# 3decomp/poissbox

Measured on AMD Instinct MI355X. Metric: CG iter/s and DoF-updates/s at 512^3; achieved HBM GB/s vs peak, higher is better.
Workload: dtype f64

## Files before the change

### include/poissbox_gpu.h

```cpp
#ifndef POISSBOX_GPU_H
#define POISSBOX_GPU_H

#include <stdint.h>

#ifdef __cplusplus
extern "C" {
#endif

#define PB_VERSION_MAJOR 0
#define PB_VERSION_MINOR 2

enum pb_error {
  PB_OK = 0,
  PB_ERR_ARG = 1,
  PB_ERR_HIP = 2,
  PB_ERR_COMM = 3,
  PB_ERR_ALLOC = 4,
  PB_ERR_UNSUPPORTED = 5,
  PB_ERR_STATE = 6
};

typedef struct pb_ctx pb_ctx;
typedef struct pb_grid pb_grid;
typedef struct pb_vec pb_vec;
// ... 181 lines not shown
int pb_solve_fgmres(pb_op* A, pb_op* P, const pb_ksp_opts* opts, const pb_ksp_fgmres_opts* fg,
                    const pb_vec* b, pb_vec* x, pb_ksp_result* res, double* history,
                    int64_t history_cap);
int pb_pc_mg_opts_default(pb_pc_mg_opts* opts);
int pb_pc_mg_opts_parse(pb_pc_mg_opts* opts, int argc, const char* const* argv);
int pb_ksp_pc_mg_set_opts(pb_ksp* ksp, const pb_pc_mg_opts* opts);
int pb_ksp_pc_mg_get_opts(const pb_ksp* ksp, pb_pc_mg_opts* opts);
int pb_solve_mg(pb_op* A, pb_op* P, const pb_ksp_opts* opts, const pb_pc_mg_opts* mg,
                const pb_vec* b, pb_vec* x, pb_ksp_result* res, double* history,
                int64_t history_cap);
int pb_ksp_chebyshev_get_eigenvalues(pb_ksp* ksp, double* emin, double* emax, int* estimated);
int pb_tridiag_extreme_eigenvalues(int n, const double* diag, const double* off, double* lo,
                                   double* hi);
int pb_ksp_pc_apply(pb_ksp* ksp, const pb_vec* r, pb_vec* z);
int pb_ksp_pc_levels(const pb_ksp* ksp, int* levels);
int pb_ksp_pc_set_coefficient_from(pb_ksp* ksp, const pb_op* C);
int pb_ksp_pc_get_coefficient_from(const pb_ksp* ksp, const pb_op** C);
int pb_ksp_guess_form(pb_ksp* ksp, const pb_vec* b, pb_vec* x);
int pb_ksp_guess_update(pb_ksp* ksp, const pb_vec* b, const pb_vec* x);
int pb_ksp_guess_reset(pb_ksp* ksp);
int pb_ksp_guess_size(const pb_ksp* ksp, int* curl, int* maxl);
int pb_solve(pb_op* A, pb_op* P, const pb_ksp_opts* opts, const pb_vec* b, pb_vec* x,
             pb_ksp_result* res, double* history, int64_t history_cap);

int pb_tdma_batched(pb_ctx* ctx, int64_t n, int64_t nbatch, int64_t line_stride,
                    int64_t elem_stride, const double* a, double* b, const double* c, double* d,
                    int periodic);
int pb_tdma_sweeps_batched(pb_ctx* ctx, int64_t n, int64_t nbatch, int64_t line_stride,
                           int64_t elem_stride, const double* a, double* b, const double* c,
                           double* d, int which);
// ... 38 lines not shown
```

### poissbox_amd/_lib.py

```python
import ctypes as C
import os
import subprocess

_HERE = os.path.dirname(os.path.abspath(__file__))
LIB_PATH = os.environ.get("PB_LIB") or os.path.join(_HERE, "libpoissbox_gpu.so")

c_i64 = C.c_int64
c_d = C.c_double
c_p = C.c_void_p
P_d = C.POINTER(C.c_double)
P_i64 = C.POINTER(C.c_int64)


class PbError(RuntimeError):
    def __init__(self, code, msg, where):
        super().__init__(f"{where} failed (code {code}): {msg}")
        self.code = code


class KspOpts(C.Structure):
    _fields_ = [("rtol", c_d), ("atol", c_d), ("dtol", c_d), ("max_it", c_i64),
                ("ksp_type", C.c_int), ("pc_type", C.c_int), ("nullspace", C.c_int),
                ("monitor", C.c_int), ("converged_reason", C.c_int), ("check_every", C.c_int),
                ("mg_levels", C.c_int), ("mg_coarse_its", C.c_int), ("sor_omega", c_d),
# ... 116 lines not shown
    "pb_ksp_fgmres_opts_default": [C.POINTER(KspFgmresOpts)],
    "pb_ksp_fgmres_opts_parse": [C.POINTER(KspFgmresOpts), C.c_int, C.POINTER(C.c_char_p)],
    "pb_ksp_fgmres_set_opts": [c_p, C.POINTER(KspFgmresOpts)],
    "pb_ksp_fgmres_get_opts": [c_p, C.POINTER(KspFgmresOpts)],
    "pb_solve_fgmres": [c_p, c_p, C.POINTER(KspOpts), C.POINTER(KspFgmresOpts), c_p, c_p,
                        C.POINTER(KspResult), P_d, c_i64],
    "pb_pc_mg_opts_default": [C.POINTER(PcMgOpts)],
    "pb_pc_mg_opts_parse": [C.POINTER(PcMgOpts), C.c_int, C.POINTER(C.c_char_p)],
    "pb_ksp_pc_mg_set_opts": [c_p, C.POINTER(PcMgOpts)],
    "pb_ksp_pc_mg_get_opts": [c_p, C.POINTER(PcMgOpts)],
    "pb_solve_mg": [c_p, c_p, C.POINTER(KspOpts), C.POINTER(PcMgOpts), c_p, c_p,
                    C.POINTER(KspResult), P_d, c_i64],
    "pb_tridiag_extreme_eigenvalues": [C.c_int, P_d, P_d, P_d, P_d],
    "pb_ksp_pc_apply": [c_p, c_p, c_p],
    "pb_ksp_pc_levels": [c_p, C.POINTER(C.c_int)],
    "pb_ksp_pc_set_coefficient_from": [c_p, c_p],
    "pb_ksp_pc_get_coefficient_from": [c_p, C.POINTER(c_p)],
    "pb_solve": [c_p, c_p, C.POINTER(KspOpts), c_p, c_p, C.POINTER(KspResult), P_d, c_i64],
    "pb_tdma_batched": [c_p, c_i64, c_i64, c_i64, c_i64, c_p, c_p, c_p, c_p, C.c_int],
    "pb_pcr_alpha_batched": [c_p, c_i64, c_i64, c_i64, c_i64, c_d, c_p],
    "pb_compact_grad": [c_p, P_d, c_p, C.POINTER(c_p)],
    "pb_compact_div": [c_p, P_d, C.POINTER(c_p), c_p],
    "pb_compact_interp": [c_p, C.c_int, c_p, c_p],
    "pb_compact_lapl": [c_p, P_d, c_p, c_p],
    "pb_compact_lapl_fast": [c_p, P_d, c_p, c_p],
    "pb_compact_grad_fast": [c_p, P_d, c_p, C.POINTER(c_p)],
    "pb_compact_div_fast": [c_p, P_d, C.POINTER(c_p), c_p],
    "pb_compact_interp_fast": [c_p, C.c_int, c_p, c_p],
    "pb_compact_1d_batched": [c_p, C.c_int, C.c_int, c_d, c_i64, c_i64, c_i64, c_i64, c_p, c_p],
    "pb_tdma_sweeps_batched": [c_p, c_i64, c_i64, c_i64, c_i64, c_p, c_p, c_p, c_p, C.c_int],
# ... 44 lines not shown
```

### poissbox_amd/api.py

```python
import ctypes as C

import numpy as np

from . import _lib as L

STAR7, COMPACT, ASSEMBLED27 = 0, 1, 2
VARCOEF = 3
COEF_ARITHMETIC, COEF_HARMONIC = 0, 1
PC_NONE, PC_JACOBI, PC_SOR, PC_MG, PC_FFT = 0, 1, 2, 3, 4
KSP_CG, KSP_PREONLY, KSP_RICHARDSON, KSP_CHEBYSHEV, KSP_FGMRES, KSP_PIPECG = 0, 1, 2, 3, 4, 5
FGMRES_REFINE_NEVER, FGMRES_REFINE_ALWAYS = 0, 2
MG_LEVELS_RICHARDSON, MG_LEVELS_CHEBYSHEV = 0, 1
KSP_NORM_DEFAULT, KSP_NORM_NONE, KSP_NORM_PRECONDITIONED = -1, 0, 1
KSP_NORM_UNPRECONDITIONED, KSP_NORM_NATURAL = 2, 3
MG_LEVELS_SOR, MG_LEVELS_JACOBI = 0, 1

REASONS = {0: "CONVERGED_ITERATING", 2: "CONVERGED_RTOL", 3: "CONVERGED_ATOL",
           4: "CONVERGED_ITS", -3: "DIVERGED_ITS", -4: "DIVERGED_DTOL",
           -8: "DIVERGED_INDEFINITE_PC", -9: "DIVERGED_NANORINF",
           -10: "DIVERGED_INDEFINITE_MAT", -5: "DIVERGED_BREAKDOWN",
           7: "CONVERGED_HAPPY_BREAKDOWN"}


def _i64_3(v):
# ... 562 lines not shown

    def chebyshev_eigenvalues(self):
        lo, hi, est = C.c_double(), C.c_double(), C.c_int()
        L.call("pb_ksp_chebyshev_get_eigenvalues", self.h, C.byref(lo), C.byref(hi), C.byref(est))
        return lo.value, hi.value, bool(est.value)

    def pc_apply(self, r, z):
        L.call("pb_ksp_pc_apply", self.h, r.h, z.h)

    @property
    def pc_levels(self):
        v = C.c_int(0)
        L.call("pb_ksp_pc_levels", self.h, C.byref(v))
        return v.value

    def pc_set_coefficient_from(self, op):
        L.call("pb_ksp_pc_set_coefficient_from", self.h, op.h if op is not None else None)
        self._pc_coef = op

    def pc_coefficient_from(self):
        h = C.c_void_p()
        L.call("pb_ksp_pc_get_coefficient_from", self.h, C.byref(h))
        if not h.value:
            return None
        op = getattr(self, "_pc_coef", None)
        assert op is not None and op.h.value == h.value
        return op

    def destroy(self):
        if self.h:
# ... 101 lines not shown
```

### poissbox_amd/csrc/pb_internal.hpp

```cpp
#pragma once

#include <hip/hip_runtime.h>
#include <rccl/rccl.h>
#include <rocprofiler-sdk-roctx/roctx.h>

#include <cstdint>
#include <cstdio>
#include <deque>
#include <map>
#include <string>
#include <functional>
#include <vector>

#include "poissbox_gpu.h"

namespace pb {

int set_error(int code, const char* fmt, ...);

#define PB_HIP(call)                                                                    \
  do {                                                                                  \
    hipError_t e_ = (call);                                                             \
    if (e_ != hipSuccess)                                                               \
      return ::pb::set_error(PB_ERR_HIP, "%s:%d %s: %s", __FILE__, __LINE__, #call,     \
// ... 248 lines not shown
int launch_mac_grad(pb_grid* g, const MacCoef& c, const double* p, double s, double* const u[3],
                    bool project, const StencilPlanes& gp, int mode);
int launch_mac_div(pb_grid* g, const MacCoef& c, double s, const double* const u[3], double* out,
                   const StencilPlanes& gp, int mode);
int launch_aij_seams(pb_grid* g, const Star& s, const double* x, const double* glo,
                     const double* ghi, double* y);
struct CgState;
int launch_mg_sor(pb_grid* g, const Star& s, double* x, const double* b, const StencilPlanes& gp,
                  double omega, int color, int first, const int* skip,
                  const CgState* sums_st = nullptr, int* nparts = nullptr);
bool sor_sweep2_supported(const pb_grid* g);
int launch_sor_sweep2(pb_grid* g, const Star& s, const double* xin, const double* b, double* xout,
                      double omega, int c1, const int* skip, const CgState* sums_st = nullptr,
                      int* nparts = nullptr);
int launch_presmooth_restrict(pb_grid* g, const Star& s, const pb_grid* cg, const double* b,
                              double* xout, double* bc, double omega, const int* skip);
int launch_post_sweep(pb_grid* g, const Star& s, const pb_grid* cg, const double* xs,
                      const double* xc, const double* b, double* xout, double omega,
                      const int* skip, const CgState* sums_st = nullptr, int* nparts = nullptr,
                      const double* xc_full = nullptr);
int launch_presmooth_residual(pb_grid* g, const Star& s, const double* b, double* x, double* res,
                              double omega, const int* skip);
int launch_mg_residual(pb_grid* g, const Star& s, const double* x, const double* b,
                       const StencilPlanes& gp, double* res, const int* skip);
int launch_mg_poly(pb_grid* g, const Star& s, const double* y, const double* yp, const double* r,
                   const double* b, double scale, double omega, double* y_out, double* r_out,
                   const int* skip);

struct CgState {
  double beta, betaold, dpi, dpiold, alpha, alpha_prev, mu, dp, ttol, rnorm0;
  double pa[3];
  double rtol, atol, dtol, dinv, ntot;
  int64_t it, its, max_it, nhist, pend_iter, pend_count;
  int64_t nlog;
  int reason, done, pc, nullspace, defer_x;
// ... 248 lines not shown
int launch_cheb_update(pb_grid* g, const Star& s, const double* y, const double* ym1,
                       const double* q, const double* b, double* y_out, double* r_out,
                       const StencilPlanes& gp, const CgState* st, double scale, bool sums,
                       int* nparts, int part_off = 0);
int launch_cheb_x(pb_grid* g, const double* y, const double* ym1, const double* q, double* y_out,
                  const CgState* st, double scale);
int launch_pre_scale_sum(pb_grid* g, const double* src, double* dst, double dinv, int* nparts);
int launch_pre_shift(pb_grid* g, double* x, double ntot);

struct Mg;
int mg_create(pb_grid* g, const double deltas[3], int pc_type, int levels_req, int coarse_its,
              double omega, Mg** out);
int mg_apply(Mg* mg, const double* r, double* z, const int* skip = nullptr,
             const CgState* sums_st = nullptr, int* nparts = nullptr);
int mg_levels(const Mg* mg);
struct MgSmoother {
  int ksp = 0, pc = 0, nu = 1;
  double rich_scale = 1.0, emin = 0.0, emax = 0.0;
};
int mg_set_smoother(Mg* mg, const MgSmoother& sm);
int mg_set_coefficient(Mg* mg, const pb_op* C);
void mg_destroy(Mg* mg);
int mg_plan_levels(const int64_t n[3], int nranks, int levels_req);

struct FftPc;
int fftpc_create(pb_grid* g, const double deltas[3], int compact, FftPc** out);
struct RUpdate {
  const double* r_in;
  const double* w;
  double* r_out;
// ... 17 lines not shown
```

### poissbox_amd/csrc/pb_mg.cpp

```cpp
#include <algorithm>
#include <cmath>

#include "pb_mg.hpp"

namespace pb {

int mg_plan_levels(const int64_t n[3], int nranks, int levels_req) {
  std::vector<int64_t> k0(nranks), nz(nranks);
  for (int r = 0; r < nranks; ++r) pb_slab_partition(n[2], nranks, r, &k0[r], &nz[r]);
  int64_t cur[3] = {n[0], n[1], n[2]};
  int L = 1;
  const int cap = levels_req > 0 ? levels_req : 64;
  while (L < cap) {
    bool ok = true;
    for (int d = 0; d < 3; ++d) ok = ok && cur[d] % 4 == 0;
    if (levels_req <= 0) ok = ok && std::min(cur[0], std::min(cur[1], cur[2])) > 4;
    for (int r = 0; r < nranks; ++r) ok = ok && k0[r] % 2 == 0 && nz[r] % 2 == 0;
    if (!ok) break;
    for (int d = 0; d < 3; ++d) cur[d] /= 2;
    for (int r = 0; r < nranks; ++r) {
      k0[r] /= 2;
      nz[r] /= 2;
    }
    ++L;
// ... 14 lines not shown
  if (mg->vmem) (void)hipFree(mg->vmem);
  if (mg->qmem) (void)hipFree(mg->qmem);
  delete mg;
}

static MgTune mg_tunings(const pb_ctx* ctx) {
  MgTune t;
  t.engine_min_plane = tune("mg_engine_min_plane", ctx->split ? 128 * 128 : 256 * 256);
  t.restrict_z_min_cols = tune("mg_restrict_z_min_cols", 4096);
  t.tail_max = tune("mg_tail_max", 8192);
  t.split_fused = tune("mg_split_fused", 1) != 0;
  t.poly_fused = tune("mg_poly_fused", 1) != 0;
  t.vc_pre_fused = tune("mg_varcoef_pre_fused", 1) != 0;
  t.vc_dinv_stored = tune("mg_varcoef_dinv_stored", 0) != 0;
  t.vc_kc = tune("mg_varcoef_kc", 0);
  return t;
}

static LevelPlan level_plan(const Mg* mg, int l, bool have_xs) {
  const MgTune& tn = mg->tn;
  const pb_grid* g = mg->lv[l].g;
  const bool split = mg->ctx->split;
  LevelPlan p;
  p.engine = g->plane >= tn.engine_min_plane;
  if (l + 1 >= (int)mg->lv.size()) return p;
  const pb_grid* c = mg->lv[l + 1].g;
  p.march = c->n[0] * c->n[1] >= tn.restrict_z_min_cols;
  if (mg->custom()) return p;
  const bool sweep2 = p.engine && sor_sweep2_supported(g);
  const bool u4 = sweep2 && (!split || (tn.split_fused && g->k0 % 2 == 0));
  if (u4 && g->nzl % 2 == 0 && (!split || g->nzl >= 3)) p.pre = LevelPlan::FusedRestrict;
  else if (sweep2) p.pre = LevelPlan::FusedResidual;
  if (u4 && have_xs && p.march && (!split || (g->nzl >= 2 && c->nzl >= 2)))
    p.post = LevelPlan::PostSweep;
  else if (sweep2 && p.march)
    p.post = LevelPlan::ProlongThenSweep2;
  return p;
}

static int tail_first(const Mg* mg) {
  const int L = (int)mg->lv.size();
  int Lt = L;
  for (int l = L - 1; l >= 1 && mg->lv[l].size() <= mg->tn.tail_max; --l) Lt = l;
  return L - Lt > kTailMax ? L : Lt;
}

static int mg_agglomerate_setup(Mg* mg) {
  pb_ctx* ctx = mg->ctx;
  const int L = (int)mg->lv.size();
  mg->La = 0;
  if (!ctx->split || L < 2 || !tune("mg_agglomerate", 1)) return PB_OK;
  if (!ctx->comm && !ctx->h_alltoallv) return PB_OK;
// ... 59 lines not shown
      lv.g = g;
      continue;
    }
    const int rc = grid_create_part(ctx, lv.n, g->L, g->k0 >> l, g->nzl >> l, &lv.g);
    if (rc != PB_OK) {
      mg_destroy(mg);
      return rc;
    }
    lv.own = true;
  }
  std::vector<double**> arrays;
  std::vector<int64_t> sizes;
  int64_t total = 0;
  for (int l = 0; l < L; ++l) {
    MgLevel& lv = mg->lv[l];
    const bool xs = level_plan(mg, l, true).post == LevelPlan::PostSweep;
    for (double** a : {l > 0 ? &lv.x : nullptr, l > 0 ? &lv.b : nullptr,
                       l < L - 1 ? &lv.res : nullptr, xs ? &lv.xs : nullptr}) {
      if (!a) continue;
      arrays.push_back(a);
      sizes.push_back(lv.g->nlocal);
      total += lv.g->nlocal;
    }
  }
  if (total > 0 && hipMalloc(&mg->mem, (size_t)total * sizeof(double)) != hipSuccess) {
    mg_destroy(mg);
    return set_error(PB_ERR_ALLOC, "multigrid levels: out of device memory");
  }
  double* p = mg->mem;
  for (size_t i = 0; i < arrays.size(); ++i) {
    *arrays[i] = p;
    p += sizes[i];
  }
  if (const int rc = mg_agglomerate_setup(mg); rc != PB_OK) {
    mg_destroy(mg);
    return rc;
  }
// ... 99 lines not shown
  *ycur = const_cast<double*>(y);
  *rcur = const_cast<double*>(r);
  return PB_OK;
}

static int down_leg(Mg* mg, int l) {
  pb_ctx* ctx = mg->ctx;
  MgLevel& F = mg->lv[l];
  MgLevel& C = mg->lv[l + 1];
  const LevelPlan& p = F.plan;
  F.cur = p.post == LevelPlan::PostSweep ? F.xs : F.x;
  double* res = F.res;
  {
    ScopedTimer t1(ctx, l == 0 ? "mg_fine_smooth_first" : "mg_coarse_levels");
    if (p.pre == LevelPlan::FusedRestrict)
      return launch_presmooth_restrict(F.g, F.s, C.g, F.b, F.cur, C.b, mg->omega, mg->skip);
    if (p.pre == LevelPlan::FusedResidual) {
      PB_TRY(launch_presmooth_residual(F.g, F.s, F.b, F.cur, F.res, mg->omega, mg->skip));
    } else if (mg->poly()) {
      PB_TRY(poly_smooth(mg, F, true, &F.cur, &res));
    } else {
      PB_TRY(level_smooth(mg, F, 0, 1));
      for (int i = 1; i < mg->sm.nu; ++i) {
        PB_TRY(level_smooth(mg, F, 0, 0));
        PB_TRY(level_smooth(mg, F, 1, 0));
      }
    }
  }
  ScopedTimer t2(ctx, l == 0 ? "mg_fine_resid_restrict" : "mg_coarse_levels");
  if (p.pre == LevelPlan::Sweeps && !mg->poly()) PB_TRY(level_residual(mg, F, F.x, res));
  return level_restrict(mg, F, res, C);
// ... 12 lines not shown

static int up_leg(Mg* mg, int l, bool from_agg, MgSums sums) {
  MgLevel& F = mg->lv[l];
  MgLevel& C = mg->lv[l + 1];
  ScopedTimer tm(mg->ctx, l == 0 ? "mg_fine_prolong_post" : "mg_coarse_levels");
  CoarsePlanes agg{C.x, nullptr, nullptr};
  if (from_agg) {
    const int64_t pc = C.g->plane, nzc = C.n[2], k0c = C.g->k0, nzl = C.g->nzl;
    const double* full = mg->ax[0];
    agg = {full + k0c * pc, full + ((k0c - 1 + nzc) % nzc) * pc, full + ((k0c + nzl) % nzc) * pc};
  }
  const CoarsePlanes* cp = from_agg ? &agg : nullptr;
  switch (F.plan.post) {
    case LevelPlan::PostSweep:
      return launch_post_sweep(F.g, F.s, C.g, F.cur, agg.xc, F.b, F.x, mg->omega, mg->skip,
                               sums.st, sums.nparts, from_agg ? mg->ax[0] : nullptr);
    case LevelPlan::ProlongThenSweep2:
      PB_TRY(level_prolong(mg, F, F.x, F.res, C, cp));
      return launch_sor_sweep2(F.g, F.s, F.res, F.b, F.x, mg->omega, 1, mg->skip, sums.st,
                               sums.nparts);
    case LevelPlan::ProlongThenHalves:
      break;
  }
  PB_TRY(level_prolong(mg, F, F.cur, F.cur, C, cp));
  if (mg->poly()) {
    double* res = nullptr;
    return poly_smooth(mg, F, false, &F.cur, &res);
  }
  for (int i = 0; i < mg->sm.nu; ++i) {
    PB_TRY(level_smooth(mg, F, 1, 0));
    PB_TRY(level_smooth(mg, F, 0, 0, i == mg->sm.nu - 1 ? sums : MgSums{}));
// ... 37 lines not shown
```

### poissbox_amd/csrc/pb_mg.hpp

```cpp
#pragma once
#include <vector>

#include "pb_internal.hpp"

namespace pb {

struct MgGeo {
  int nx, ny, nzl;
  int64_t plane, nlocal, k0;
};

struct LevelPlan {
  enum Pre { FusedRestrict, FusedResidual, Sweeps };
  enum Post { PostSweep, ProlongThenSweep2, ProlongThenHalves };
  bool engine = false;
  Pre pre = Sweeps;
  Post post = ProlongThenHalves;
  bool march = false;
};

struct MgLevel {
  int64_t n[3];
  double h[3];
  Star s;
  pb_grid* g = nullptr;
  bool own = false;
  double* x = nullptr;
  double* b = nullptr;
  double* res = nullptr;
  double* xs = nullptr;
  double* t1 = nullptr;
  double* t2 = nullptr;
  double* r2 = nullptr;
  const double* beta = nullptr;
  double* beta_own = nullptr;
  double* dinv = nullptr;
  double* q = nullptr;
  double qs = 0.0;
  Star vs;
  LevelPlan plan;
  double* cur = nullptr;
  int64_t size() const { return n[0] * n[1] * n[2]; }
  MgGeo geo() const {
    return MgGeo{(int)g->n[0], (int)g->n[1], (int)g->nzl, g->plane, g->nlocal, g->k0};
  }
};

struct MgTune {
  int64_t engine_min_plane;
  int64_t restrict_z_min_cols;
  int64_t tail_max;
  bool split_fused;
  bool poly_fused;
  bool vc_pre_fused, vc_dinv_stored;
  int vc_kc;
};

struct MgSums {
  const CgState* st = nullptr;
  int* nparts = nullptr;
};

struct CoarsePlanes {
  const double *xc, *lo, *hi;
};

static constexpr int kTailMax = 12;

struct Mg {
  pb_ctx* ctx = nullptr;
// ... 41 lines not shown
```

### poissbox_amd/csrc/pb_mg_sweep.hip

```cpp
#include <algorithm>
#include <type_traits>

#include "pb_device.hpp"

namespace pb {

#ifndef PB_SWEEP2_TY
#define PB_SWEEP2_TY 3
#endif
static constexpr int kTY2 = PB_SWEEP2_TY;
static constexpr int kRW = kTY2 + 4;
static constexpr int kSegOut = 112;
static constexpr int kSegLead = 4;

__device__ __forceinline__ double pick(bool e1, const double (&v)[2]) {
  const long long m = -(long long)e1;
  return __builtin_bit_cast(double, (__builtin_bit_cast(long long, v[1]) & m) |
                                        (__builtin_bit_cast(long long, v[0]) & ~m));
}

struct Sweep2Geo {
  int nx, ny, nzl;
  int64_t plane;
  int nseg, ntile, kc, nchunk;
// ... 362 lines not shown
      rq[0][r] = rq[1][r];
      rq[1][r] = rq[2][r];
      rq[2][r] = rn[r];
#pragma unroll
      for (int e = 0; e < 2; ++e) {
        s1[0][r][e] = s1[1][r][e];
        s1[1][r][e] = s1[2][r][e];
        bq[0][r][e] = bq[1][r][e];
        bq[1][r][e] = bq[2][r][e];
      }
    }
    keepb(nraw, bq[2]);
  }
}

template <int NW, int TY>
__device__ __forceinline__ void presmooth_restrict_u4_range(
    const Sweep2Geo& g, int ncx, int64_t cplane, double cx, double cy, double cz, double cc,
    double omega, const double* __restrict__ b, double* __restrict__ xout,
    double* __restrict__ bc, int seg, int tile, int kb, int ke, double (&xch)[2][8][NW][64]) {
  static_assert(TY % 2 == 0 && TY >= 2, "whole coarse rows per wave");
  constexpr int RB = NW * TY;
  constexpr int LO = 4;
  constexpr int SB = RB - 2 * LO;
  constexpr int NCR = TY / 2;
  const double icc = 1.0 / cc;
  const int lane = threadIdx.x & 63, wid = __builtin_amdgcn_readfirstlane(threadIdx.x >> 6);
  const int nx = g.nx, ny = g.ny, nz = g.nzl;
  if (kb >= nz) return;
  const int g0 = tile * SB - LO;
  const int br0 = wid * TY;
// ... 144 lines not shown
          a = a + cy * yp;
          a = a + cz * s1p[r][e];
          rv[e] = bq0[r][e] - a;
        }
        const double rlo = dpp_from_lower(rv[1]);
        const double rhi = dpp_from_upper(rv[0]);
        double sx = w[0] * rlo;
        sx = sx + w[1] * rv[0];
        sx = sx + w[2] * rv[1];
        sx = sx + w[3] * rhi;
        sxc[r] = sx;
      }
      if (k >= kb && k < ke && out_ok) {
        const int64_t base = (int64_t)k * g.plane;
#pragma unroll
        for (int r = 0; r < TY; ++r)
          if (row_ok >> r & 1u) store_row<2>(xout, rix(base + ro[r]), s1c[r], g.nt);
      }
    } else {
#pragma unroll
      for (int r = 0; r < TY; ++r) sxc[r] = 0.0;
    }
    xch[KP][6][wid][lane] = sxc[0];
    xch[KP][7][wid][lane] = sxc[TY - 1];
    const int kr = k - 1;
    if (kr >= kb - 1) {
#pragma unroll
      for (int c = 0; c < NCR; ++c) {
        double sy = 0.0;
#pragma unroll
        for (int bb = 0; bb < 4; ++bb) {
          const int r = 2 * c - 1 + bb;
// ... 36 lines not shown
    return;
  }
  const int k0 = T * W, h = g.nzl - k0;
  if (h <= 0) return;
  const int64_t total = (int64_t)ncol * h;
  const int64_t e = min(total, (int64_t)(bid - T * ncol + 1) * W);
  for (int64_t s = (int64_t)(bid - T * ncol) * W; s < e;) {
    const int col = (int)(s / h);
    const int kb = (int)(s - (int64_t)col * h);
    const int ke = (int)min((int64_t)h, kb + (e - s));
    fn(col, k0 + kb, k0 + ke);
    s += ke - kb;
  }
}

template <int NW, int TY>
__global__ __launch_bounds__(64 * NW) void presmooth_restrict_u4_kernel(
    Sweep2Geo g, int ncx, int64_t cplane, double cx, double cy, double cz, double cc,
    double omega, const double* __restrict__ b, double* __restrict__ xout,
    double* __restrict__ bc, const int* skip) {
  __shared__ double xch[2][8][NW][64];
  if (skip && *skip) return;
  int bid = xcd_block(g.remap);
  if (g.wsplit > 0) {
    split_ranges(g, bid, [&](int col, int kb, int ke) {
      presmooth_restrict_u4_range<NW, TY>(g, ncx, cplane, cx, cy, cz, cc, omega, b, xout, bc,
                                          col % g.nseg, col / g.nseg, kb, ke, xch);
      __syncthreads();
    });
    return;
  }
  const int seg = bid % g.nseg;
  bid /= g.nseg;
  const int tile = bid % g.ntile;
  const int chunk = bid / g.ntile;
  const int kb = chunk * g.kc;
  presmooth_restrict_u4_range<NW, TY>(g, ncx, cplane, cx, cy, cz, cc, omega, b, xout, bc, seg,
                                      tile, kb, min(kb + g.kc, g.nzl), xch);
}

struct PostGeo {
  int ncx, ncy, ncz;
  int64_t cplane;
  int split;
  const double* cgh[4];
};

template <bool SUMS, int NW, int TY>
__device__ __forceinline__ void post_sweep_u4_range(
    const Sweep2Geo& g, const PostGeo& cgeo, double cx, double cy, double cz, double cc,
    double omega, const double* __restrict__ xs, const double* __restrict__ xc,
    const double* __restrict__ b, double* __restrict__ xout, double mu, int seg, int tile, int kb,
    int ke, double (&xch)[2][6][NW][64], double (&acc)[4]) {
  static_assert(TY % 2 == 0 && TY >= 2, "own rows start on an even fine row");
  constexpr int RB = NW * TY;
  constexpr int SB = RB - 4;
  constexpr int NC = TY / 2 + 2;
  const double icc = 1.0 / cc;
  const int lane = threadIdx.x & 63, wid = __builtin_amdgcn_readfirstlane(threadIdx.x >> 6);
  const int nx = g.nx, ny = g.ny, nz = g.nzl;
  if (kb < nz) {
    const int g0 = tile * SB - 2;
    const int br0 = wid * TY;
// ... 14 lines not shown
    }
    const unsigned boff = (unsigned)ip * 8u;
    auto rix = [&](int64_t row) { return RowIx{row, boff}; };
    auto wrapk = [&](int kk) { kk %= nz; return kk < 0 ? kk + nz : kk; };
    auto pl = [&](int kk) -> int64_t { return (int64_t)wrapk(kk) * g.plane; };
    int64_t crow[NC];
#pragma unroll
    for (int t = 0; t < NC; ++t) crow[t] = (int64_t)wrap((j0 >> 1) - 1 + t, cgeo.ncy) * cgeo.ncx;
    const unsigned cboff = (unsigned)(ip >> 1) * 8u;
    auto xsplane = [&](int kk) -> const double* {
      if (!g.split) return xs + pl(kk);
      if (kk >= 0 && kk < nz) return xs + (int64_t)kk * g.plane;
      const int gi = kk < 0 ? max(kk + 2, 0) : 2 + min(kk - nz, 1);
      return g.xg + (int64_t)gi * g.plane;
    };
    auto ldx = [&](double (&dst)[TY + 2][2], int kk) {
      const double* src = xsplane(kk);
#pragma unroll
      for (int r = 0; r < TY; ++r) load_row<2>(src, rix(ro[r]), dst[r + 1]);
    };
    auto ldc = [&](double (&cv)[NC], int K) {
      const double* cp;
      if (!cgeo.split) {
        K %= cgeo.ncz;
        if (K < 0) K += cgeo.ncz;
        cp = xc + (int64_t)K * cgeo.cplane;
      } else if (K >= 0 && K < cgeo.ncz) {
        cp = xc + (int64_t)K * cgeo.cplane;
      } else {
        const int gi = K < 0 ? max(K + 2, 0) : 2 + min(K - cgeo.ncz, 1);
        cp = cgeo.cgh[gi];
      }
#pragma unroll
      for (int t = 0; t < NC; ++t)
// ... 98 lines not shown
    };
    double XQ[2][TY + 2][2];
    double XM[2][TY];
    double S1[4][TY];
    double SH[2][2];
    double BB[2][TY];
    double BB1[2][SUMS ? TY : 1];
    double YC[2][TY][2];
    const int K0 = kb >> 1;
    {
      double cv[NC];
      ldc(cv, K0 - 2);
      yinterp(cv, YC[0]);
      ldc(cv, K0 - 1);
      yinterp(cv, YC[1]);
      ldx(XQ[1], kb - 2);
      prolong(XQ[1], YC[1], YC[0]);
#pragma unroll
      for (int r = 0; r < TY; ++r) XM[1][r] = XQ[1][r + 1][e1(r, 0) ^ 1];
      ldc(cv, K0);
      yinterp(cv, YC[0]);
      ldx(XQ[0], kb - 1);
      prolong(XQ[0], YC[1], YC[0]);
      put_x(1, XQ[0]);
    }
#pragma unroll
    for (int r = 0; r < TY; ++r) {
      XM[0][r] = BB[0][r] = BB[1][r] = 0.0;
      S1[0][r] = S1[1][r] = S1[2][r] = 0.0;
      if constexpr (SUMS) BB1[0][r] = BB1[1][r] = 0.0;
    }
    SH[0][0] = SH[0][1] = 0.0;
    auto body = [&](auto Qc, int k) {
      constexpr int Q = decltype(Qc)::value;
      constexpr int KP = Q & 1;
      double (&xq1)[TY + 2][2] = XQ[Q & 1];
      double (&xq2)[TY + 2][2] = XQ[(Q + 1) & 1];
      double (&xm)[TY] = XM[Q & 1];
      double (&x0)[TY] = XM[(Q + 1) & 1];
      double (&bm)[TY] = BB[Q & 1];
      double (&bm1)[SUMS ? TY : 1] = BB1[Q & 1];
      double (&shp)[2] = SH[Q & 1];
      double (&shc)[2] = SH[(Q + 1) & 1];
      constexpr int KN = Q >> 1;
      double bq1[TY][2], cv[NC];
      ldx(xq2, k + 2);
      if constexpr (Q & 1) ldc(cv, ((k + 2) >> 1) + 1);
      ldb(bq1, k + 1);
      __syncthreads();
      {
        constexpr int rp = KP ^ 1;
        xq1[0][0] = xch[rp][2][wm][lane];
        xq1[0][1] = xch[rp][3][wm][lane];
        xq1[TY + 1][0] = xch[rp][0][wp][lane];
        xq1[TY + 1][1] = xch[rp][1][wp][lane];
        shc[0] = xch[rp][5][wm][lane];
        shc[1] = xch[rp][4][wp][lane];
      }
      if (k > kb && k <= ke)
        half2(std::integral_constant<int, KP ^ 1>{}, k - 1, S1[Q], S1[(Q + 1) & 3],
              S1[(Q + 2) & 3], shp, xm, bm, bm1);
      if constexpr (Q & 1) yinterp(cv, YC[KN ^ 1]);
      prolong(xq2, YC[KN], YC[KN ^ 1]);
      put_x(KP, xq2);
      double (&s1n)[TY] = S1[(Q + 3) & 3];
      half1(std::integral_constant<int, KP ^ 1>{}, x0, xq1, xq2, bq1, s1n);
      xch[KP][4][wid][lane] = s1n[0];
      xch[KP][5][wid][lane] = s1n[TY - 1];
#pragma unroll
      for (int r = 0; r < TY; ++r) {
        const int e = e1(r, KP ^ 1);
        xm[r] = xq1[r + 1][e ^ 1];
        bm[r] = bq1[r][e ^ 1];
        if constexpr (SUMS) bm1[r] = bq1[r][e];
      }
    };
#pragma unroll 1
    for (int k = kb - 2; k <= ke; k += 4) {
      body(std::integral_constant<int, 0>{}, k);
      body(std::integral_constant<int, 1>{}, k + 1);
      body(std::integral_constant<int, 2>{}, k + 2);
      body(std::integral_constant<int, 3>{}, k + 3);
    }
  }
}

template <bool SUMS, int NW, int TY>
__global__ __launch_bounds__(64 * NW) void post_sweep_u4_kernel(
    Sweep2Geo g, PostGeo cgeo, double cx, double cy, double cz, double cc, double omega,
    const double* __restrict__ xs, const double* __restrict__ xc, const double* __restrict__ b,
    double* __restrict__ xout, const CgState* st, double* parts, const int* skip) {
  __shared__ double xch[2][6][NW][64];
  if (skip && *skip) return;
  double acc[4] = {0.0, 0.0, 0.0, 0.0};
  const double mu = SUMS ? st->mu : 0.0;
  int bid = xcd_block(g.remap);
  if (g.wsplit > 0) {
    split_ranges(g, bid, [&](int col, int kb, int ke) {
      post_sweep_u4_range<SUMS, NW, TY>(g, cgeo, cx, cy, cz, cc, omega, xs, xc, b, xout, mu,
                                        col % g.nseg, col / g.nseg, kb, ke, xch, acc);
      __syncthreads();
    });
  } else {
    const int seg = bid % g.nseg;
    bid /= g.nseg;
    const int tile = bid % g.ntile;
    const int chunk = bid / g.ntile;
    const int kb = chunk * g.kc;
    post_sweep_u4_range<SUMS, NW, TY>(g, cgeo, cx, cy, cz, cc, omega, xs, xc, b, xout, mu, seg,
                                      tile, kb, min(kb + g.kc, g.nzl), xch, acc);
  }
  if constexpr (SUMS) block_partials<4>(acc, parts);
}

bool sor_sweep2_supported(const pb_grid* g) {
  return g->n[0] >= 128 && g->n[0] % 2 == 0 && g->n[1] % 2 == 0 && g->n[1] >= 8 &&
         g->nzl >= 4 && tune("mg_sweep2", 1) != 0;
}

static int ensure_ghost2(pb_grid* g) {
  if (!g->ghost2 && hipMalloc(&g->ghost2, 6 * (size_t)g->plane * sizeof(double)) != hipSuccess)
    return set_error(PB_ERR_ALLOC, "deep ghost planes: out of device memory");
  return PB_OK;
}
// ... 88 lines not shown
  if (cg->n[0] * 2 != g->n[0] || cg->n[1] * 2 != g->n[1] || cg->nzl * 2 != g->nzl)
    return set_error(PB_ERR_ARG, "%s: coarse grid is not half the fine one", what);
  if (g->ctx->split && (g->nzl < min_planes || cg->nzl < 2))
    return set_error(PB_ERR_UNSUPPORTED, "%s", thin);
  if (g->k0 % 2 != 0) return set_error(PB_ERR_UNSUPPORTED, "%s: odd slab origin", what);
  sweep2_geo(g, geo);
  geo.split = 0;
  geo.xg = geo.bg_lo = geo.bg_hi = nullptr;
  geo.ntile = (geo.ny + rows - 1) / rows;
  return PB_OK;
}

int launch_post_sweep(pb_grid* g, const Star& s, const pb_grid* cg, const double* xs,
                      const double* xc, const double* b, double* xout, double omega,
                      const int* skip, const CgState* sums_st, int* nparts,
                      const double* xc_full) {
  ScopedTimer tm(g->ctx, "mg_post_sweep");
  const bool split = g->ctx->split;
  if (xs == xout) return set_error(PB_ERR_ARG, "fused post-smoothing must run out of place");
  constexpr int nw = 8, ty = 4;
  Sweep2Geo geo;
  PB_TRY(u4_setup("fused post-smoothing", g, cg, 2, "fused post-smoothing: slabs of < 2 planes",
                  nw * ty - 4, geo));
  PostGeo cgeo{(int)cg->n[0], (int)cg->n[1], (int)cg->nzl, cg->plane, 0,
                {nullptr, nullptr, nullptr, nullptr}};
  if (split) {
    pb_grid* gc = const_cast<pb_grid*>(cg);
    PB_TRY(ensure_ghost2(g));
    PB_TRY(ensure_ghost2(gc));
    PB_TRY(halo_exchange_n(g, xs, xs + (g->nzl - 2) * g->plane, 2, g->ghost2,
                           g->ghost2 + 2 * g->plane));
    PB_TRY(halo_exchange(g, b, b + (g->nzl - 1) * g->plane));
    geo.split = 1;
    geo.xg = g->ghost2;
// ... 9 lines not shown
    } else {
      PB_TRY(halo_exchange_n(gc, xc, xc + (gc->nzl - 2) * gc->plane, 2, gc->ghost2,
                             gc->ghost2 + 2 * gc->plane));
      for (int i = 0; i < 4; ++i) cgeo.cgh[i] = gc->ghost2 + (int64_t)i * gc->plane;
    }
  }
  const int columns = geo.nseg * geo.ntile;
  const int target = 8 * g->ctx->num_cus;
  int nchunk = std::max(1, (target + columns - 1) / columns);
  const int minz = std::min(64, std::max(16, geo.nzl / 8));
  nchunk = std::min(nchunk, std::max(1, geo.nzl / minz));
  int64_t nblocks = set_chunks(geo, nchunk, 4);
  nblocks = balanced_split(g, geo, std::max(0, tune("mg_u4_split", 0)), 4, nblocks);
  double* parts;
  PB_TRY(sums_parts(g, sums_st, nblocks, nparts, &parts));
  auto kern = sums_st ? post_sweep_u4_kernel<true, nw, ty> : post_sweep_u4_kernel<false, nw, ty>;
  hipLaunchKernelGGL(kern, dim3((unsigned)nblocks), dim3(64 * nw), 0, g->ctx->stream, geo, cgeo,
                     s.cx, s.cy, s.cz, s.cc, omega, xs, xc, b, xout, sums_st, parts, skip);
  PB_HIP(hipGetLastError());
  return PB_OK;
}

int launch_presmooth_restrict(pb_grid* g, const Star& s, const pb_grid* cg, const double* b,
                              double* xout, double* bc, double omega, const int* skip) {
  ScopedTimer tm(g->ctx, "mg_presmooth_restrict");
  const bool split = g->ctx->split;
  if (b == xout) return set_error(PB_ERR_ARG, "fused pre-smoothing must run out of place");
  if (!sor_sweep2_supported(g) || g->nzl % 2)
    return set_error(PB_ERR_UNSUPPORTED, "fused restriction: grid not supported");
  constexpr int nw = 8, ty = 4;
  Sweep2Geo geo;
  PB_TRY(u4_setup("fused restriction", g, cg, 3,
                  "fused restriction on N ranks: >= 3 planes per slab", nw * ty - 8, geo));
  if (split) {
    PB_TRY(ensure_ghost2(g));
    PB_TRY(halo_exchange_n(g, b, b + (g->nzl - 3) * g->plane, 3, g->ghost2,
                           g->ghost2 + 3 * g->plane));
    geo.split = 1;
    geo.xg = g->ghost2;
  }
  const int columns = geo.nseg * geo.ntile;
  int nchunk = std::max(1, g->ctx->num_cus / columns);
  if (geo.nzl / nchunk < 128) nchunk = std::max(1, (4 * g->ctx->num_cus + columns - 1) / columns);
  nchunk = std::min(nchunk, std::max(1, geo.nzl / 16));
  int64_t nblocks = set_chunks(geo, nchunk, 2);
  const int ps = tune("mg_u4_split", -1);
  nblocks = balanced_split(g, geo, ps >= 0 ? ps : (nblocks > g->ctx->num_cus ? 1 : 0), 2,
                           nblocks);
  hipLaunchKernelGGL((presmooth_restrict_u4_kernel<nw, ty>), dim3((unsigned)nblocks),
                     dim3(64 * nw), 0, g->ctx->stream, geo, (int)cg->n[0], cg->plane, s.cx, s.cy,
                     s.cz, s.cc, omega, b, xout, bc, skip);
  PB_HIP(hipGetLastError());
  return PB_OK;
}

int launch_presmooth_residual(pb_grid* g, const Star& s, const double* b, double* x, double* res,
                              double omega, const int* skip) {
  ScopedTimer tm(g->ctx, "mg_presmooth_residual");
  if (b == x || b == res || x == res)
    return set_error(PB_ERR_ARG, "fused pre-smoothing + residual must run out of place");
  Sweep2Geo geo;
  const int64_t nblocks = sweep2_geo(g, geo);
  PB_TRY(sweep2_ghosts(g, b, b, geo));
  auto kern = geo.split ? presmooth_resid_kernel<true> : presmooth_resid_kernel<false>;
  hipLaunchKernelGGL(kern, dim3((unsigned)nblocks), dim3(kThreads), 0, g->ctx->stream, geo,
                     s.cx, s.cy, s.cz, s.cc, omega, b, x, res, skip);
// ... 6 lines not shown
```

### poissbox_amd/csrc/pb_runtime.cpp

```cpp
#include <time.h>

#include <algorithm>
#include <atomic>
#include <chrono>
#include <cstdarg>
#include <cstdlib>
#include <cstring>
#include <condition_variable>
#include <memory>
#include <mutex>
#include <string>
#include <thread>
#include <unordered_map>

#include "pb_internal.hpp"

namespace pb {

hipError_t field_alloc(void** p, size_t bytes) { return hipMalloc(p, bytes); }

void field_free(void* p) {
  if (p) (void)hipFree(p);
}

namespace {
const char* const kTuneNames[] = {
    "a2a_copy_self", "cg_defer_x", "engine_kc_skew", "cg_fold", "cg_fuse", "cg_sr_fused", "cheb_fused", "comm_mark_every",
    "comm_stall_test_ms", "compact_lines", "fft_rupd", "fgmres_fused", "pipecg_fused", "fft_zpad", "fft_zpad_min_plane",
    "force_comm", "ksp_lazy0", "mac_wgcu", "mg_agglomerate", "mg_engine_min_plane", "mg_poly_fused", "mg_restrict_z_min_cols",
    "mg_split_fused", "mg_sweep2", "mg_tail_max", "mg_u4_split", "mg_varcoef_dinv_stored", "mg_varcoef_kc",
    "mg_varcoef_pre_fused", "pcr_lines", "rich_fused", "sor_omega_any", "sr_ddiff",
    "stencil_kc", "stencil_kc_skew", "stencil_nt", "stencil_tall", "stencil_wgcu", "varcoef_dot_fused", "varcoef_wgcu", "x_dot_cu"};
constexpr int kNumTune = (int)(sizeof(kTuneNames) / sizeof(kTuneNames[0]));
std::atomic<int> g_tune_val[kNumTune];
std::atomic<int> g_tune_set[kNumTune];
std::atomic<int> g_tune_nset{0};
int tune_index(const char* name) {
  for (int i = 0; i < kNumTune; ++i)
    if (strcmp(kTuneNames[i], name) == 0) return i;
  return -1;
}
}

int tune(const char* name, int dflt) {
  if (g_tune_nset.load(std::memory_order_acquire) == 0) return dflt;
  const int i = tune_index(name);
// ... 1017 lines not shown
```

### poissbox_amd/csrc/pb_solver.cpp

```cpp
#include <cmath>
#include <cstdio>
#include <cstring>
#include <string>
#include <vector>

#include "pb_ksp.hpp"

using namespace pb;

int pb::ensure_done_cap(pb_ksp* k, int64_t need) {
  if (need <= k->done_cap) return PB_OK;
  int64_t cap = need < 1024 ? 1024 : need * 2;
  int* h = nullptr;
  PB_HIP(hipHostMalloc(&h, (size_t)cap * sizeof(int), hipHostMallocMapped));
  memset(h, 0, (size_t)cap * sizeof(int));
  if (k->h_done) {
    PB_TRY(wait_stream(k->A->grid->ctx, k->A->grid->ctx->stream, "KSP flag buffer"));
    memcpy(h, k->h_done, (size_t)k->done_cap * sizeof(int));
    (void)hipHostFree(k->h_done);
  }
  k->h_done = h;
  PB_HIP(hipHostGetDevicePointer((void**)&k->h_done_dev, h, 0));
  k->done_cap = cap;
  return PB_OK;
// ... 332 lines not shown
    PB_HIP(hipMemcpyAsync(z->d, r->d, (size_t)g->nlocal * sizeof(double),
                          hipMemcpyDeviceToDevice, ctx->stream));
    if (k->opts.pc_type == PB_PC_JACOBI)
      PB_TRY(vec_update(ctx, 2, z->d, nullptr, g->nlocal, 1.0 / k->P->cc));
  }
  PB_SYNC(ctx, "pb_ksp_pc_apply");
  return PB_OK;
}

int pb_ksp_pc_levels(const pb_ksp* k, int* levels) {
  PB_CHECK_ARG(k && levels, "bad args");
  *levels = k->mg ? mg_levels(k->mg) : 0;
  return PB_OK;
}

int pb_ksp_pc_mg_set_opts(pb_ksp* k, const pb_pc_mg_opts* o) {
  PB_CHECK_ARG(k && o, "bad args");
  if (k->opts.pc_type != PB_PC_MG || !k->mg)
    return set_error(PB_ERR_STATE, "KSP created without -pc_type mg");
  if (k->begun) return set_error(PB_ERR_STATE, "pb_ksp_pc_mg_set_opts inside a solve");
  PB_TRY(check_mg_opts(o));
  if (k->coef && o->levels_pc_type == PB_MG_LEVELS_JACOBI)
    return set_error(PB_ERR_UNSUPPORTED,
                     "a Jacobi-type level smoother with pb_ksp_pc_set_coefficient_from: the "
                     "variable-coefficient levels smooth with -mg_levels_pc_type sor");
  MgSmoother sm;
  sm.ksp = o->levels_ksp_type;
  sm.pc = o->levels_pc_type;
  sm.nu = o->levels_ksp_max_it;
  sm.rich_scale = o->levels_richardson_scale;
// ... 84 lines not shown
```

Measured before the change: 102.4 billion.

## Store only black-colour half of pre-smoothed x between fused MG sweeps

```diff
diff --git a/include/poissbox_gpu.h b/include/poissbox_gpu.h
--- a/include/poissbox_gpu.h
+++ b/include/poissbox_gpu.h
@@ -219,6 +219,7 @@
                                    double* hi);
 int pb_ksp_pc_apply(pb_ksp* ksp, const pb_vec* r, pb_vec* z);
 int pb_ksp_pc_levels(const pb_ksp* ksp, int* levels);
+int pb_ksp_pc_mg_xs_half(const pb_ksp* ksp, unsigned* level_mask);
 int pb_ksp_pc_set_coefficient_from(pb_ksp* ksp, const pb_op* C);
 int pb_ksp_pc_get_coefficient_from(const pb_ksp* ksp, const pb_op** C);
 int pb_ksp_guess_form(pb_ksp* ksp, const pb_vec* b, pb_vec* x);
diff --git a/poissbox_amd/_lib.py b/poissbox_amd/_lib.py
--- a/poissbox_amd/_lib.py
+++ b/poissbox_amd/_lib.py
@@ -154,6 +154,7 @@
     "pb_tridiag_extreme_eigenvalues": [C.c_int, P_d, P_d, P_d, P_d],
     "pb_ksp_pc_apply": [c_p, c_p, c_p],
     "pb_ksp_pc_levels": [c_p, C.POINTER(C.c_int)],
+    "pb_ksp_pc_mg_xs_half": [c_p, C.POINTER(C.c_uint)],
     "pb_ksp_pc_set_coefficient_from": [c_p, c_p],
     "pb_ksp_pc_get_coefficient_from": [c_p, C.POINTER(c_p)],
     "pb_solve": [c_p, c_p, C.POINTER(KspOpts), c_p, c_p, C.POINTER(KspResult), P_d, c_i64],
diff --git a/poissbox_amd/api.py b/poissbox_amd/api.py
--- a/poissbox_amd/api.py
+++ b/poissbox_amd/api.py
@@ -600,6 +600,12 @@
         L.call("pb_ksp_pc_levels", self.h, C.byref(v))
         return v.value
 
+    @property
+    def pc_mg_xs_half_levels(self):
+        v = C.c_uint(0)
+        L.call("pb_ksp_pc_mg_xs_half", self.h, C.byref(v))
+        return [l for l in range(32) if v.value >> l & 1]
+
     def pc_set_coefficient_from(self, op):
         L.call("pb_ksp_pc_set_coefficient_from", self.h, op.h if op is not None else None)
         self._pc_coef = op
diff --git a/poissbox_amd/csrc/pb_internal.hpp b/poissbox_amd/csrc/pb_internal.hpp
--- a/poissbox_amd/csrc/pb_internal.hpp
+++ b/poissbox_amd/csrc/pb_internal.hpp
@@ -286,11 +286,12 @@
                       double omega, int c1, const int* skip, const CgState* sums_st = nullptr,
                       int* nparts = nullptr);
 int launch_presmooth_restrict(pb_grid* g, const Star& s, const pb_grid* cg, const double* b,
-                              double* xout, double* bc, double omega, const int* skip);
+                              double* xout, double* bc, double omega, const int* skip,
+                              bool xs_half = false);
 int launch_post_sweep(pb_grid* g, const Star& s, const pb_grid* cg, const double* xs,
                       const double* xc, const double* b, double* xout, double omega,
                       const int* skip, const CgState* sums_st = nullptr, int* nparts = nullptr,
-                      const double* xc_full = nullptr);
+                      const double* xc_full = nullptr, bool xs_half = false);
 int launch_presmooth_residual(pb_grid* g, const Star& s, const double* b, double* x, double* res,
                               double omega, const int* skip);
 int launch_mg_residual(pb_grid* g, const Star& s, const double* x, const double* b,
@@ -569,6 +570,7 @@
 int mg_apply(Mg* mg, const double* r, double* z, const int* skip = nullptr,
              const CgState* sums_st = nullptr, int* nparts = nullptr);
 int mg_levels(const Mg* mg);
+unsigned mg_xs_half_levels(Mg* mg);
 struct MgSmoother {
   int ksp = 0, pc = 0, nu = 1;
   double rich_scale = 1.0, emin = 0.0, emax = 0.0;
diff --git a/poissbox_amd/csrc/pb_mg.cpp b/poissbox_amd/csrc/pb_mg.cpp
--- a/poissbox_amd/csrc/pb_mg.cpp
+++ b/poissbox_amd/csrc/pb_mg.cpp
@@ -52,6 +52,7 @@
   t.vc_pre_fused = tune("mg_varcoef_pre_fused", 1) != 0;
   t.vc_dinv_stored = tune("mg_varcoef_dinv_stored", 0) != 0;
   t.vc_kc = tune("mg_varcoef_kc", 0);
+  t.xs_half = tune("mg_xs_half", 1) != 0;
   return t;
 }
 
@@ -73,7 +74,21 @@
     p.post = LevelPlan::PostSweep;
   else if (sweep2 && p.march)
     p.post = LevelPlan::ProlongThenSweep2;
+  const MgLevel& lv = mg->lv[l];
+  const bool half = tn.xs_half && !split && p.pre == LevelPlan::FusedRestrict &&
+                    p.post == LevelPlan::PostSweep;
+  p.xs_half = half && (!lv.xs || lv.xs_half);
+  if (lv.xs && lv.xs_half && !half && p.post == LevelPlan::PostSweep)
+    p.post = LevelPlan::ProlongThenSweep2;
   return p;
+}
+
+unsigned mg_xs_half_levels(Mg* mg) {
+  mg->tn = mg_tunings(mg->ctx);
+  unsigned mask = 0;
+  for (int l = 0; l < (int)mg->lv.size() && l < 32; ++l)
+    if (level_plan(mg, l, mg->lv[l].xs != nullptr).xs_half) mask |= 1u << l;
+  return mask;
 }
 
 static int tail_first(const Mg* mg) {
@@ -163,13 +178,16 @@
   int64_t total = 0;
   for (int l = 0; l < L; ++l) {
     MgLevel& lv = mg->lv[l];
-    const bool xs = level_plan(mg, l, true).post == LevelPlan::PostSweep;
+    const LevelPlan plan = level_plan(mg, l, true);
+    const bool xs = plan.post == LevelPlan::PostSweep;
+    lv.xs_half = xs && plan.xs_half;
     for (double** a : {l > 0 ? &lv.x : nullptr, l > 0 ? &lv.b : nullptr,
                        l < L - 1 ? &lv.res : nullptr, xs ? &lv.xs : nullptr}) {
       if (!a) continue;
+      const int64_t len = a == &lv.xs && lv.xs_half ? lv.g->nlocal / 2 : lv.g->nlocal;
       arrays.push_back(a);
-      sizes.push_back(lv.g->nlocal);
-      total += lv.g->nlocal;
+      sizes.push_back(len);
+      total += len;
     }
   }
   if (total > 0 && hipMalloc(&mg->mem, (size_t)total * sizeof(double)) != hipSuccess) {
@@ -299,7 +317,8 @@
   {
     ScopedTimer t1(ctx, l == 0 ? "mg_fine_smooth_first" : "mg_coarse_levels");
     if (p.pre == LevelPlan::FusedRestrict)
-      return launch_presmooth_restrict(F.g, F.s, C.g, F.b, F.cur, C.b, mg->omega, mg->skip);
+      return launch_presmooth_restrict(F.g, F.s, C.g, F.b, F.cur, C.b, mg->omega, mg->skip,
+                                       p.xs_half);
     if (p.pre == LevelPlan::FusedResidual) {
       PB_TRY(launch_presmooth_residual(F.g, F.s, F.b, F.cur, F.res, mg->omega, mg->skip));
     } else if (mg->poly()) {
@@ -342,7 +361,8 @@
   switch (F.plan.post) {
     case LevelPlan::PostSweep:
       return launch_post_sweep(F.g, F.s, C.g, F.cur, agg.xc, F.b, F.x, mg->omega, mg->skip,
-                               sums.st, sums.nparts, from_agg ? mg->ax[0] : nullptr);
+                               sums.st, sums.nparts, from_agg ? mg->ax[0] : nullptr,
+                               F.plan.xs_half);
     case LevelPlan::ProlongThenSweep2:
       PB_TRY(level_prolong(mg, F, F.x, F.res, C, cp));
       return launch_sor_sweep2(F.g, F.s, F.res, F.b, F.x, mg->omega, 1, mg->skip, sums.st,
diff --git a/poissbox_amd/csrc/pb_mg.hpp b/poissbox_amd/csrc/pb_mg.hpp
--- a/poissbox_amd/csrc/pb_mg.hpp
+++ b/poissbox_amd/csrc/pb_mg.hpp
@@ -17,6 +17,7 @@
   Pre pre = Sweeps;
   Post post = ProlongThenHalves;
   bool march = false;
+  bool xs_half = false;
 };
 
 struct MgLevel {
@@ -29,6 +30,7 @@
   double* b = nullptr;
   double* res = nullptr;
   double* xs = nullptr;
+  bool xs_half = false;
   double* t1 = nullptr;
   double* t2 = nullptr;
   double* r2 = nullptr;
@@ -54,6 +56,7 @@
   bool poly_fused;
   bool vc_pre_fused, vc_dinv_stored;
   int vc_kc;
+  bool xs_half;
 };
 
 struct MgSums {
diff --git a/poissbox_amd/csrc/pb_mg_sweep.hip b/poissbox_amd/csrc/pb_mg_sweep.hip
--- a/poissbox_amd/csrc/pb_mg_sweep.hip
+++ b/poissbox_amd/csrc/pb_mg_sweep.hip
@@ -400,7 +400,7 @@
   }
 }
 
-template <int NW, int TY>
+template <int NW, int TY, bool XH>
 __device__ __forceinline__ void presmooth_restrict_u4_range(
     const Sweep2Geo& g, int ncx, int64_t cplane, double cx, double cy, double cz, double cc,
     double omega, const double* __restrict__ b, double* __restrict__ xout,
@@ -575,8 +575,15 @@
       if (k >= kb && k < ke && out_ok) {
         const int64_t base = (int64_t)k * g.plane;
 #pragma unroll
-        for (int r = 0; r < TY; ++r)
-          if (row_ok >> r & 1u) store_row<2>(xout, rix(base + ro[r]), s1c[r], g.nt);
+        for (int r = 0; r < TY; ++r) {
+          if (!(row_ok >> r & 1u)) continue;
+          if constexpr (XH) {
+            const double hv[1] = {s1c[r][1 - red_e(r, KP)]};
+            store_row<1>(xout, RowIx{(base + ro[r]) >> 1, boff >> 1}, hv, g.nt);
+          } else {
+            store_row<2>(xout, rix(base + ro[r]), s1c[r], g.nt);
+          }
+        }
       }
     } else {
 #pragma unroll
@@ -643,7 +650,7 @@
   }
 }
 
-template <int NW, int TY>
+template <int NW, int TY, bool XH>
 __global__ __launch_bounds__(64 * NW) void presmooth_restrict_u4_kernel(
     Sweep2Geo g, int ncx, int64_t cplane, double cx, double cy, double cz, double cc,
     double omega, const double* __restrict__ b, double* __restrict__ xout,
@@ -653,7 +660,7 @@
   int bid = xcd_block(g.remap);
   if (g.wsplit > 0) {
     split_ranges(g, bid, [&](int col, int kb, int ke) {
-      presmooth_restrict_u4_range<NW, TY>(g, ncx, cplane, cx, cy, cz, cc, omega, b, xout, bc,
+      presmooth_restrict_u4_range<NW, TY, XH>(g, ncx, cplane, cx, cy, cz, cc, omega, b, xout, bc,
                                           col % g.nseg, col / g.nseg, kb, ke, xch);
       __syncthreads();
     });
@@ -664,7 +671,7 @@
   const int tile = bid % g.ntile;
   const int chunk = bid / g.ntile;
   const int kb = chunk * g.kc;
-  presmooth_restrict_u4_range<NW, TY>(g, ncx, cplane, cx, cy, cz, cc, omega, b, xout, bc, seg,
+  presmooth_restrict_u4_range<NW, TY, XH>(g, ncx, cplane, cx, cy, cz, cc, omega, b, xout, bc, seg,
                                       tile, kb, min(kb + g.kc, g.nzl), xch);
 }
 
@@ -675,7 +682,7 @@
   const double* cgh[4];
 };
 
-template <bool SUMS, int NW, int TY>
+template <bool SUMS, int NW, int TY, bool XH>
 __device__ __forceinline__ void post_sweep_u4_range(
     const Sweep2Geo& g, const PostGeo& cgeo, double cx, double cy, double cz, double cc,
     double omega, const double* __restrict__ xs, const double* __restrict__ xc,
@@ -720,10 +727,37 @@
       const int gi = kk < 0 ? max(kk + 2, 0) : 2 + min(kk - nz, 1);
       return g.xg + (int64_t)gi * g.plane;
     };
-    auto ldx = [&](double (&dst)[TY + 2][2], int kk) {
-      const double* src = xsplane(kk);
-#pragma unroll
-      for (int r = 0; r < TY; ++r) load_row<2>(src, rix(ro[r]), dst[r + 1]);
+    auto ldx = [&](auto Pc, double (&dst)[TY + 2][2], int kk) {
+      if constexpr (XH) {
+        constexpr int P = decltype(Pc)::value;
+        const int64_t po = pl(kk);
+        const double* src = xs + (po >> 1);
+        const double* bs = b + po;
+#pragma unroll
+        for (int r = 0; r < TY; ++r) {
+          const int er = (r + P) & 1;
+          double hv[1];
+          load_row<1>(src, RowIx{ro[r] >> 1, boff >> 1}, hv);
+          dst[r + 1][er ^ 1] = hv[0];
+          load_row<1>(bs, RowIx{ro[r], boff + 8u * er}, hv);
+          dst[r + 1][er] = hv[0];
+        }
+      } else {
+        const double* src = xsplane(kk);
+#pragma unroll
+        for (int r = 0; r < TY; ++r) load_row<2>(src, rix(ro[r]), dst[r + 1]);
+      }
+    };
+    auto mkred = [&](auto Pc, double (&v)[TY + 2][2]) {
+      if constexpr (XH) {
+        constexpr int P = decltype(Pc)::value;
+#pragma unroll
+        for (int r = 0; r < TY; ++r) {
+          const int er = (r + P) & 1;
+          const double t = (v[r + 1][er] - 0.0) * icc;
+          v[r + 1][er] = (1.0 - omega) * 0.0 + omega * t;
+        }
+      }
     };
     auto ldc = [&](double (&cv)[NC], int K) {
       const double* cp;
@@ -852,13 +886,15 @@
       yinterp(cv, YC[0]);
       ldc(cv, K0 - 1);
       yinterp(cv, YC[1]);
-      ldx(XQ[1], kb - 2);
+      ldx(std::integral_constant<int, 0>{}, XQ[1], kb - 2);
+      mkred(std::integral_constant<int, 0>{}, XQ[1]);
       prolong(XQ[1], YC[1], YC[0]);
 #pragma unroll
       for (int r = 0; r < TY; ++r) XM[1][r] = XQ[1][r + 1][e1(r, 0) ^ 1];
       ldc(cv, K0);
       yinterp(cv, YC[0]);
-      ldx(XQ[0], kb - 1);
+      ldx(std::integral_constant<int, 1>{}, XQ[0], kb - 1);
+      mkred(std::integral_constant<int, 1>{}, XQ[0]);
       prolong(XQ[0], YC[1], YC[0]);
       put_x(1, XQ[0]);
     }
@@ -882,7 +918,7 @@
       double (&shc)[2] = SH[(Q + 1) & 1];
       constexpr int KN = Q >> 1;
       double bq1[TY][2], cv[NC];
-      ldx(xq2, k + 2);
+      ldx(std::integral_constant<int, KP>{}, xq2, k + 2);
       if constexpr (Q & 1) ldc(cv, ((k + 2) >> 1) + 1);
       ldb(bq1, k + 1);
       __syncthreads();
@@ -899,6 +935,7 @@
         half2(std::integral_constant<int, KP ^ 1>{}, k - 1, S1[Q], S1[(Q + 1) & 3],
               S1[(Q + 2) & 3], shp, xm, bm, bm1);
       if constexpr (Q & 1) yinterp(cv, YC[KN ^ 1]);
+      mkred(std::integral_constant<int, KP>{}, xq2);
       prolong(xq2, YC[KN], YC[KN ^ 1]);
       put_x(KP, xq2);
       double (&s1n)[TY] = S1[(Q + 3) & 3];
@@ -923,7 +960,7 @@
   }
 }
 
-template <bool SUMS, int NW, int TY>
+template <bool SUMS, int NW, int TY, bool XH>
 __global__ __launch_bounds__(64 * NW) void post_sweep_u4_kernel(
     Sweep2Geo g, PostGeo cgeo, double cx, double cy, double cz, double cc, double omega,
     const double* __restrict__ xs, const double* __restrict__ xc, const double* __restrict__ b,
@@ -935,7 +972,7 @@
   int bid = xcd_block(g.remap);
   if (g.wsplit > 0) {
     split_ranges(g, bid, [&](int col, int kb, int ke) {
-      post_sweep_u4_range<SUMS, NW, TY>(g, cgeo, cx, cy, cz, cc, omega, xs, xc, b, xout, mu,
+      post_sweep_u4_range<SUMS, NW, TY, XH>(g, cgeo, cx, cy, cz, cc, omega, xs, xc, b, xout, mu,
                                         col % g.nseg, col / g.nseg, kb, ke, xch, acc);
       __syncthreads();
     });
@@ -945,7 +982,7 @@
     const int tile = bid % g.ntile;
     const int chunk = bid / g.ntile;
     const int kb = chunk * g.kc;
-    post_sweep_u4_range<SUMS, NW, TY>(g, cgeo, cx, cy, cz, cc, omega, xs, xc, b, xout, mu, seg,
+    post_sweep_u4_range<SUMS, NW, TY, XH>(g, cgeo, cx, cy, cz, cc, omega, xs, xc, b, xout, mu, seg,
                                       tile, kb, min(kb + g.kc, g.nzl), xch, acc);
   }
   if constexpr (SUMS) block_partials<4>(acc, parts);
@@ -1064,10 +1101,12 @@
 int launch_post_sweep(pb_grid* g, const Star& s, const pb_grid* cg, const double* xs,
                       const double* xc, const double* b, double* xout, double omega,
                       const int* skip, const CgState* sums_st, int* nparts,
-                      const double* xc_full) {
+                      const double* xc_full, bool xs_half) {
   ScopedTimer tm(g->ctx, "mg_post_sweep");
   const bool split = g->ctx->split;
   if (xs == xout) return set_error(PB_ERR_ARG, "fused post-smoothing must run out of place");
+  if (xs_half && split)
+    return set_error(PB_ERR_UNSUPPORTED, "fused post-smoothing: half-size x_s on a split grid");
   constexpr int nw = 8, ty = 4;
   Sweep2Geo geo;
   PB_TRY(u4_setup("fused post-smoothing", g, cg, 2, "fused post-smoothing: slabs of < 2 planes",
@@ -1107,7 +1146,10 @@
   nblocks = balanced_split(g, geo, std::max(0, tune("mg_u4_split", 0)), 4, nblocks);
   double* parts;
   PB_TRY(sums_parts(g, sums_st, nblocks, nparts, &parts));
-  auto kern = sums_st ? post_sweep_u4_kernel<true, nw, ty> : post_sweep_u4_kernel<false, nw, ty>;
+  auto kern = xs_half ? (sums_st ? post_sweep_u4_kernel<true, nw, ty, true>
+                                 : post_sweep_u4_kernel<false, nw, ty, true>)
+                      : (sums_st ? post_sweep_u4_kernel<true, nw, ty, false>
+                                 : post_sweep_u4_kernel<false, nw, ty, false>);
   hipLaunchKernelGGL(kern, dim3((unsigned)nblocks), dim3(64 * nw), 0, g->ctx->stream, geo, cgeo,
                      s.cx, s.cy, s.cz, s.cc, omega, xs, xc, b, xout, sums_st, parts, skip);
   PB_HIP(hipGetLastError());
@@ -1115,10 +1157,13 @@
 }
 
 int launch_presmooth_restrict(pb_grid* g, const Star& s, const pb_grid* cg, const double* b,
-                              double* xout, double* bc, double omega, const int* skip) {
+                              double* xout, double* bc, double omega, const int* skip,
+                              bool xs_half) {
   ScopedTimer tm(g->ctx, "mg_presmooth_restrict");
   const bool split = g->ctx->split;
   if (b == xout) return set_error(PB_ERR_ARG, "fused pre-smoothing must run out of place");
+  if (xs_half && split)
+    return set_error(PB_ERR_UNSUPPORTED, "fused restriction: half-size x_s on a split grid");
   if (!sor_sweep2_supported(g) || g->nzl % 2)
     return set_error(PB_ERR_UNSUPPORTED, "fused restriction: grid not supported");
   constexpr int nw = 8, ty = 4;
@@ -1140,9 +1185,10 @@
   const int ps = tune("mg_u4_split", -1);
   nblocks = balanced_split(g, geo, ps >= 0 ? ps : (nblocks > g->ctx->num_cus ? 1 : 0), 2,
                            nblocks);
-  hipLaunchKernelGGL((presmooth_restrict_u4_kernel<nw, ty>), dim3((unsigned)nblocks),
-                     dim3(64 * nw), 0, g->ctx->stream, geo, (int)cg->n[0], cg->plane, s.cx, s.cy,
-                     s.cz, s.cc, omega, b, xout, bc, skip);
+  auto kern = xs_half ? presmooth_restrict_u4_kernel<nw, ty, true>
+                      : presmooth_restrict_u4_kernel<nw, ty, false>;
+  hipLaunchKernelGGL(kern, dim3((unsigned)nblocks), dim3(64 * nw), 0, g->ctx->stream, geo,
+                     (int)cg->n[0], cg->plane, s.cx, s.cy, s.cz, s.cc, omega, b, xout, bc, skip);
   PB_HIP(hipGetLastError());
   return PB_OK;
 }
diff --git a/poissbox_amd/csrc/pb_runtime.cpp b/poissbox_amd/csrc/pb_runtime.cpp
--- a/poissbox_amd/csrc/pb_runtime.cpp
+++ b/poissbox_amd/csrc/pb_runtime.cpp
@@ -29,7 +29,7 @@
     "comm_stall_test_ms", "compact_lines", "fft_rupd", "fgmres_fused", "pipecg_fused", "fft_zpad", "fft_zpad_min_plane",
     "force_comm", "ksp_lazy0", "mac_wgcu", "mg_agglomerate", "mg_engine_min_plane", "mg_poly_fused", "mg_restrict_z_min_cols",
     "mg_split_fused", "mg_sweep2", "mg_tail_max", "mg_u4_split", "mg_varcoef_dinv_stored", "mg_varcoef_kc",
-    "mg_varcoef_pre_fused", "pcr_lines", "rich_fused", "sor_omega_any", "sr_ddiff",
+    "mg_varcoef_pre_fused", "mg_xs_half", "pcr_lines", "rich_fused", "sor_omega_any", "sr_ddiff",
     "stencil_kc", "stencil_kc_skew", "stencil_nt", "stencil_tall", "stencil_wgcu", "varcoef_dot_fused", "varcoef_wgcu", "x_dot_cu"};
 constexpr int kNumTune = (int)(sizeof(kTuneNames) / sizeof(kTuneNames[0]));
 std::atomic<int> g_tune_val[kNumTune];
diff --git a/poissbox_amd/csrc/pb_solver.cpp b/poissbox_amd/csrc/pb_solver.cpp
--- a/poissbox_amd/csrc/pb_solver.cpp
+++ b/poissbox_amd/csrc/pb_solver.cpp
@@ -370,6 +370,12 @@
   return PB_OK;
 }
 
+int pb_ksp_pc_mg_xs_half(const pb_ksp* k, unsigned* level_mask) {
+  PB_CHECK_ARG(k && level_mask, "bad args");
+  *level_mask = k->mg ? mg_xs_half_levels(k->mg) : 0u;
+  return PB_OK;
+}
+
 int pb_ksp_pc_mg_set_opts(pb_ksp* k, const pb_pc_mg_opts* o) {
   PB_CHECK_ARG(k && o, "bad args");
   if (k->opts.pc_type != PB_PC_MG || !k->mg)
```

After: 102.4 billion. No clear change (-0.0%).
